# saiprasadbarke/robustmvd

Hardware: AMD Instinct MI355X
Metric: depth-maps/sec at 768x1152x4srcx256planes; warp+aggregate HBM GB/s vs roofline (higher is better)
Workload: dtype f32; 1 GPU; mvsnet (Path B) forward 768x1152, 4 source views, 256 planes, batch 1 per step (BASELINE.json configs[2]); the regulariser's two layers with 32 input channels (conv0, conv4): every fp32 operand as two range-scaled fp16 terms on fp16 MFMA, fp32 accumulation (at least as close to a float64 convolution as the fp32 matrix instruction over 1e-42..1e30: tests/test_hip_f16.py), the other nine layers and ; parallelism=1 independent replica(s), frames round-robin, no collectives

## Files before the change

### robustmvd_amd/csrc/conv2d_split.hip

```cpp
#include "mvd_common.h"
#include <algorithm>
#include <stdlib.h>

#ifndef C2_KO
#define C2_KO 0
#endif

namespace mvd {

typedef _Float16 c2h8 __attribute__((ext_vector_type(8)));
typedef float c2f4 __attribute__((ext_vector_type(4)));
typedef unsigned int c2u4 __attribute__((ext_vector_type(4)));
constexpr int C2_TH = 16, C2_TW = 16;

template <int KH, int KW, int S, int U8, bool IMG = false>
struct C2Geom {
    static constexpr int CC = 8 * U8;
    static constexpr int PB = 16;
    static constexpr int PH = (C2_TH - 1) * S + KH, PW = (C2_TW - 1) * S + KW;
    static constexpr int PWS = (PW + S - 1) / S;
    static constexpr int ROWB = S * S * PWS * PB;
    static constexpr int C8S = (PH * S * PWS * PB + 255) / 256 * 256;
    static constexpr int PLANE = U8 * C8S;
    static constexpr int UNITS = KH * KW * U8;
// ... 313 lines not shown
                xh = yh; xl = yl;
                if (m + 2 < MTW && !(C2_KO & 8)) {
                    yh = *reinterpret_cast<const c2h8*>(a + (m + 2) * G::ROWB);
                    yl = *reinterpret_cast<const c2h8*>(a + (m + 2) * G::ROWB + PLANE);
                }
#pragma unroll
                for (int t = 0; t < NTW; ++t) {
                    if (C2_KO & 2) {
                        acc[m][t][0] += (float)ch[0] * (float)wh[t][0] + (float)cl[1] * (float)wl[t][1];
                        continue;
                    }
                    acc[m][t] = __builtin_amdgcn_mfma_f32_16x16x32_f16(wh[t], ch, acc[m][t], 0, 0, 0);
                    acc[m][t] = __builtin_amdgcn_mfma_f32_16x16x32_f16(wl[t], ch, acc[m][t], 0, 0, 0);
                    acc[m][t] = __builtin_amdgcn_mfma_f32_16x16x32_f16(wh[t], cl, acc[m][t], 0, 0, 0);
                }
                __builtin_amdgcn_sched_barrier(0);
            }
#pragma unroll
            for (int t = 0; t < NTW; ++t) { wh[t] = nh[t]; wl[t] = nl[t]; }
        }
    }

    const int ox = ox0 + px16;
    float amax = 0.f;
#pragma unroll
    for (int t = 0; t < NTW; ++t) {
        const int cb = (nt0 + t) * 16 + 4 * g;
        if (p.part) {
            if (ox < p.Wo)
#pragma unroll
                for (int m = 0; m < MTW; ++m) {
                    const int oy = oy0 + wm * MTW + m;
                    if (oy >= p.Ho) continue;
                    const size_t pl = ((size_t)b * p.Ho + oy) * p.Wo + ox;
                    *reinterpret_cast<c2f4*>(p.part + (((size_t)cls * p.ksplit + ks) * p.B * p.Ho * p.Wo + pl) * p.ncp + cb) = acc[m][t];
                }
            continue;
        }
        if (cb >= p.Cout || ((C2_KO & 16) && p.B > 1000)) continue;
        const C2Chan kc = c2_chan(p, cb, xsc_inv);
        if (ox < p.Wo) {
            const size_t o0 = c2_out_offset(p, bb, od, oy0 + wm * MTW, ox, cls, cb), ostep = c2_row_step(p);
#pragma unroll
            for (int m = 0; m < MTW; ++m)
                if (oy0 + wm * MTW + m < p.Ho) c2_finish(p, o0 + m * ostep, cb, acc[m][t], kc, amax);
        }
    }
    if (p.yamax && !p.part) {
        for (int o = 32; o > 0; o >>= 1) amax = fmaxf(amax, __shfl_xor(amax, o));
        if (lane == 0) wmax[wv] = amax;
        __syncthreads();
        if (tid == 0) {
            amax = fmaxf(fmaxf(wmax[0], wmax[1]), fmaxf(wmax[2], wmax[3]));
            raise_absmax_seen(p.yamax, amax, amax_seen);
        }
    }
}

__global__ void __launch_bounds__(256) c2_reduce_kernel(C2Params p) {
    __shared__ float wmax[4];
    const int npix = p.B * p.Ho * p.Wo;
    const int c4n = (p.Cout + 3) / 4;
    const int cls = blockIdx.y;
    float xsc_inv;
    {
        const unsigned mb = __float_as_uint(*p.xamax);
        const int ex = (int)((mb >> 23) & 0xffu) - 127;
        const int e = max(-125, min(125, ex - 14));
        xsc_inv = __uint_as_float((unsigned)(127 + e) << 23);
    }
    float amax = 0.f;
    for (int i = blockIdx.x * 256 + threadIdx.x; i < npix * c4n; i += gridDim.x * 256) {
        const int pl = i / c4n;
        const int cb = (i - pl * c4n) * 4;
        const float* pp = p.part + ((size_t)cls * p.ksplit * npix + pl) * p.ncp + cb;
        const size_t kstr = (size_t)npix * p.ncp;
        c2f4 s = c2f4{0, 0, 0, 0};
        int ks = 0;
        for (; ks + 8 <= p.ksplit; ks += 8) {
            c2f4 v[8];
#pragma unroll
            for (int q = 0; q < 8; ++q) v[q] = *reinterpret_cast<const c2f4*>(pp + (size_t)(ks + q) * kstr);
#pragma unroll
            for (int q = 0; q < 8; ++q) s += v[q];
        }
        for (; ks + 2 <= p.ksplit; ks += 2) {
            const c2f4 v0 = *reinterpret_cast<const c2f4*>(pp + (size_t)ks * kstr), v1 = *reinterpret_cast<const c2f4*>(pp + (size_t)(ks + 1) * kstr);
            s += v0;
            s += v1;
        }
        const int row = pl / p.Wo, ox = pl - row * p.Wo, b = row / p.Ho, oy = row - b * p.Ho;
        const int bb = p.Do == 1 ? b : b / p.Do, od = b - bb * p.Do;
        c2_finish(p, c2_out_offset(p, bb, od, oy, ox, cls, cb), cb, s, c2_chan(p, cb, xsc_inv), amax);
    }
    if (p.yamax) {
        for (int o = 32; o > 0; o >>= 1) amax = fmaxf(amax, __shfl_xor(amax, o));
        if ((threadIdx.x & 63) == 0) wmax[threadIdx.x >> 6] = amax;
        __syncthreads();
        if (threadIdx.x == 0) {
            amax = fmaxf(fmaxf(wmax[0], wmax[1]), fmaxf(wmax[2], wmax[3]));
            raise_absmax(p.yamax, amax);
        }
    }
}

__global__ void __launch_bounds__(256) upsample2x_nhwc_kernel(const float* __restrict__ x, float* __restrict__ y, float* yamax, int B, int C, int h,
                                                              int w, int ys) {
    __shared__ float wmax[4];
    const long long n = (long long)B * 4 * h * w;
    float amax = 0.f;
    for (long long i = (long long)blockIdx.x * 256 + threadIdx.x; i < n; i += (long long)gridDim.x * 256) {
        const int ox = (int)(i % (2 * w)), oy = (int)((i / (2 * w)) % (2 * h)), b = (int)(i / (4LL * h * w));
        const float sy = fmaxf(0.5f * ((float)oy + 0.5f) - 0.5f, 0.f), sx = fmaxf(0.5f * ((float)ox + 0.5f) - 0.5f, 0.f);
        const int y0 = (int)sy, x0 = (int)sx;
        const int y1 = y0 + (y0 < h - 1 ? 1 : 0), x1 = x0 + (x0 < w - 1 ? 1 : 0);
        const float ly1 = sy - (float)y0, ly0 = 1.f - ly1, lx1 = sx - (float)x0, lx0 = 1.f - lx1;
        for (int c = 0; c < C; ++c) {
            const float* pl = x + ((size_t)b * C + c) * h * w;
            const float v = ly0 * (lx0 * pl[(size_t)y0 * w + x0] + lx1 * pl[(size_t)y0 * w + x1]) +
                            ly1 * (lx0 * pl[(size_t)y1 * w + x0] + lx1 * pl[(size_t)y1 * w + x1]);
            y[(size_t)i * ys + c] = v;
            amax = fmaxf(amax, finite_abs_or_zero(v));
        }
    }
    if (yamax) {
        for (int o = 32; o > 0; o >>= 1) amax = fmaxf(amax, __shfl_xor(amax, o));
        if ((threadIdx.x & 63) == 0) wmax[threadIdx.x >> 6] = amax;
        __syncthreads();
        if (threadIdx.x == 0) {
            amax = fmaxf(fmaxf(wmax[0], wmax[1]), fmaxf(wmax[2], wmax[3]));
            raise_absmax(yamax, amax);
        }
    }
}

__device__ __forceinline__ int c3_deconv_kidx(int a, int t) { return a == 0 ? (t == 0 ? 1 : -1) : (t == 0 ? 2 : 0); }

__global__ void c3_pack_kernel(const float* __restrict__ w, const float* __restrict__ eun, _Float16* __restrict__ packed, int Cin, int Cout,
                               int U8, int nchunks_c, int ntiles, int steps, int transposed, long long total) {
    const long long e = (long long)blockIdx.x * 256 + threadIdx.x;
    if (e >= total) return;
    const int KD = transposed ? 2 : 3, KP = transposed ? 2 : 3;
    const int j = (int)(e & 7), lane = (int)((e >> 3) & 63), term = (int)((e >> 9) & 1);
    long long r = e >> 10;
    const int step = (int)(r % steps); r /= steps;
    const int chunk = (int)(r % (KD * nchunks_c)); r /= KD * nchunks_c;
    const int nt = (int)r;
    const int kd = chunk / nchunks_c, cc = chunk % nchunks_c;
    const int ce = nt * 16 + (lane & 15), unit = 4 * step + (lane >> 4);
    const int tap = unit / U8, cin = cc * 8 * U8 + 8 * (unit % U8) + j;
    const int ncout = transposed ? 8 * Cout : Cout;
    float v = 0.f;
    if (tap < KP * KP && cin < Cin && ce < ncout) {
        const int ty = tap / KP, tx = tap % KP;
        if (transposed) {
            const int k3 = ce / Cout, c = ce % Cout;
            const int kz = c3_deconv_kidx(k3 >> 2, kd), ky = c3_deconv_kidx((k3 >> 1) & 1, ty), kx = c3_deconv_kidx(k3 & 1, tx);
            if (kz >= 0 && ky >= 0 && kx >= 0) v = w[((((size_t)cin * Cout + c) * 3 + kz) * 3 + ky) * 3 + kx];
        } else {
            v = w[((((size_t)ce * Cin + cin) * 3 + kd) * 3 + ty) * 3 + tx];
        }
        v = v / eun[ce];
    }
    const _Float16 hi = (_Float16)v;
    packed[e] = term == 0 ? hi : (_Float16)(v - (float)hi);
}

__global__ void c3_wscale_kernel(const float* __restrict__ w, float* __restrict__ eun, int Cin, int Cout, int transposed, int ncout, int cpad) {
    __shared__ float red[256];
    const int ce = blockIdx.x, c = ce % Cout;
    float m = 0.f;
    if (ce < ncout)
        for (int e = threadIdx.x; e < Cin * 27; e += 256) {
            const int ci = e / 27, t = e % 27;
            const float v = fabsf(transposed ? w[((size_t)ci * Cout + c) * 27 + t] : w[((size_t)c * Cin + ci) * 27 + t]);
            m = (v <= 3.4e38f && v > m) ? v : m;
        }
    red[threadIdx.x] = m;
    __syncthreads();
    for (int o = 128; o > 0; o >>= 1) {
        if (threadIdx.x < o) red[threadIdx.x] = fmaxf(red[threadIdx.x], red[threadIdx.x + o]);
        __syncthreads();
    }
    if (threadIdx.x == 0 && ce < cpad) {
        const int ex = (int)((__float_as_uint(red[0]) >> 23) & 0xffu) - 127;
        const int k = red[0] > 0.f ? max(-100, min(100, ex - 10)) : 0;
        eun[ce] = ldexpf(1.0f, k);
    }
}

struct C2Shape {
    int KH, KW, S, U8, steps;
    bool transposed, nchw3;
};

static bool c2_shape(int KH, int KW, int stride, int mode, int cin_pad, C2Shape* s) {
    s->transposed = mode == 1;
    s->nchw3 = mode == 2;
    s->KH = KH; s->KW = KW; s->S = stride;
    if (mode == 1) {
        if (KH != 4 || KW != 4 || stride != 2 || cin_pad % 32) return false;
        s->KH = s->KW = 2; s->S = 1; s->U8 = 4;
    } else if (mode == 2) {
        if (KH != 7 || KW != 7 || stride != 2 || cin_pad != 8) return false;
        s->U8 = 1;
        s->steps = 7;
        return true;
    } else if (KH == 1 && KW == 1 && stride == 1) {
        if (cin_pad % 32) return false;
        s->U8 = 4;
    } else if (KH == 3 && KW == 3 && stride == 1) {
        s->U8 = cin_pad % 32 == 0 ? 4 : 1;
    } else if ((KH == 3 && KW == 3 && stride == 2) || (KH == 5 && KW == 5 && stride == 2)) {
        s->U8 = 1;
    } else {
        return false;
    }
    if (cin_pad % (8 * s->U8)) return false;
    s->steps = (s->KH * s->KW * s->U8 + 3) / 4;
    return true;
}

static int c2_bn(int cout) {
    if (const char* e = exp_env("MVD_C2_BN")) {
        const int v = atoi(e);
        if (v == 16 || v == 32 || v == 64 || v == 128) return v;
    }
    return cout > 64 ? 128 : cout > 32 ? 64 : cout > 16 ? 32 : 16;
}
static int c2_ntiles(int cout) { return (cout + c2_bn(cout) - 1) / c2_bn(cout) * (c2_bn(cout) / 16); }
static size_t c2_frag_bytes(const C2Shape& s, int cin_pad, int cout) {
    const size_t nchunks = (size_t)cin_pad / (8 * s.U8);
    return (s.transposed ? 4 : 1) * (size_t)c2_ntiles(cout) * nchunks * s.steps * 2048;
}
static int c2_cpad(int cout) { return (cout + 127) / 128 * 128; }

struct C2Plan {
    int Ho, Wo, tiles_x, tiles_y, bn, nblocks, ncp, ncls, nchunks, ksplit;
    long long tiles;
    size_t part_bytes;
};
static C2Plan c2_plan(const C2Shape& s, int B, int Hi, int Wi, int cin_pad, int cout, int KH, int KW, int stride) {
    C2Plan q{};
    if (s.transposed) { q.Ho = Hi; q.Wo = Wi; q.ncls = 4; }
    else { q.Ho = (Hi + 2 * (KH / 2) - KH) / stride + 1; q.Wo = (Wi + 2 * (KW / 2) - KW) / stride + 1; q.ncls = 1; }
    q.tiles_y = (q.Ho + C2_TH - 1) / C2_TH;
    q.tiles_x = (q.Wo + C2_TW - 1) / C2_TW;
    q.bn = c2_bn(cout);
    q.nblocks = (cout + q.bn - 1) / q.bn;
    q.ncp = q.nblocks * q.bn;
    q.nchunks = cin_pad / (8 * s.U8);
    q.tiles = (long long)q.tiles_x * q.tiles_y * B * q.nblocks * q.ncls;
    q.ksplit = 1;
    if (q.tiles < 128)
        while (q.tiles * q.ksplit < 320 && q.ksplit < 32 && q.nchunks / (q.ksplit * 2) >= 2) q.ksplit *= 2;
    if (const char* e = exp_env("MVD_C2_KSPLIT")) {
        const int v = atoi(e);
        if (v >= 1 && v <= 32 && (v & (v - 1)) == 0 && v <= q.nchunks) q.ksplit = v;
    }
    q.part_bytes = q.ksplit > 1 ? (size_t)q.ksplit * q.ncls * B * q.Ho * q.Wo * q.ncp * sizeof(float) : 0;
    return q;
}

template <int KH, int KW, int S, int U8, int WM, int NTW, bool NCHW3>
static int c2_launch(const C2Params& p, long long nblk, hipStream_t st) {
    using G = C2Geom<KH, KW, S, U8, NCHW3>;
    auto kern = conv2d_split_kernel<KH, KW, S, U8, WM, NTW, NCHW3>;
    constexpr int lds = 2 * G::PLANE + 16;
    static_assert(lds <= 80 * 1024, "two workgroups per CU");
    if (lds > 48 * 1024 && hipFuncSetAttribute((const void*)kern, hipFuncAttributeMaxDynamicSharedMemorySize, lds) != hipSuccess)
        return launch_status("conv2d_split: LDS attribute");
    hipLaunchKernelGGL(kern, dim3((unsigned)nblk), dim3(256), lds, st, p);
    return launch_status("conv2d_split");
}

template <int KH, int KW, int S, int U8, bool NCHW3>
static int c2_launch_bn(const C2Params& p, int bn, long long nblk, hipStream_t st) {
    switch (bn) {
        case 128: return c2_launch<KH, KW, S, U8, 1, 2, NCHW3>(p, nblk, st);
        case 64: return c2_launch<KH, KW, S, U8, 1, 1, NCHW3>(p, nblk, st);
        case 32: return c2_launch<KH, KW, S, U8, 2, 1, NCHW3>(p, nblk, st);
        case 16: return c2_launch<KH, KW, S, U8, 4, 1, NCHW3>(p, nblk, st);
    }
    return MVD_ERR_INVALID_ARG;
}

static int c2_dispatch(const C2Shape& s, const C2Params& p, int bn, long long nblk, hipStream_t st) {
    if (s.nchw3) return c2_launch_bn<7, 7, 2, 1, true>(p, bn, nblk, st);
    if (s.KH == 1) return c2_launch_bn<1, 1, 1, 4, false>(p, bn, nblk, st);
    if (s.KH == 2) return s.U8 == 4 ? c2_launch_bn<2, 2, 1, 4, false>(p, bn, nblk, st) : c2_launch_bn<2, 2, 1, 2, false>(p, bn, nblk, st);
    if (s.KH == 5) return c2_launch_bn<5, 5, 2, 1, false>(p, bn, nblk, st);
    if (s.S == 2) return c2_launch_bn<3, 3, 2, 1, false>(p, bn, nblk, st);
    if (s.U8 == 4) return c2_launch_bn<3, 3, 1, 4, false>(p, bn, nblk, st);
    return c2_launch_bn<3, 3, 1, 1, false>(p, bn, nblk, st);
}

}

extern "C" {

size_t mvd_conv2d_split_packed_weight_bytes(int Cin_pad, int Cout, int KH, int KW, int stride, int mode) {
    mvd::C2Shape s;
    if (Cin_pad <= 0 || Cout <= 0 || !mvd::c2_shape(KH, KW, stride, mode, Cin_pad, &s)) return 0;
    return mvd::c2_frag_bytes(s, Cin_pad, Cout) + (size_t)mvd::c2_cpad(Cout) * sizeof(float);
}

int mvd_pack_conv2d_weights_split(const float* w, int Cin, int Cin_pad, int Cout, int KH, int KW, int stride, int mode, void* packed,
                                  mvd_stream_t stream) {
    MVD_REQUIRE(w && packed, "pack_conv2d_weights_split: NULL argument");
    mvd::C2Shape s;
    MVD_REQUIRE(Cin > 0 && Cin <= Cin_pad && Cout > 0 && mvd::c2_shape(KH, KW, stride, mode, Cin_pad, &s),
                "pack_conv2d_weights_split: layer %dx%d stride %d mode %d with %d (padded %d) -> %d channels is not built", KH, KW, stride, mode,
                Cin, Cin_pad, Cout);
    hipStream_t st = (hipStream_t)stream;
    const size_t fb = mvd::c2_frag_bytes(s, Cin_pad, Cout);
    float* eun = reinterpret_cast<float*>(static_cast<char*>(packed) + fb);
    const int cpad = mvd::c2_cpad(Cout);
    hipLaunchKernelGGL(mvd::c2_wscale_kernel, dim3(cpad), dim3(256), 0, st, w, eun, Cin, Cout, KH * KW, s.transposed ? 1 : 0, cpad);
    const long long total = (long long)(fb / 2);
    hipLaunchKernelGGL(mvd::c2_pack_kernel, dim3((unsigned)((total + 255) / 256)), dim3(256), 0, st, w, eun, (_Float16*)packed, Cin, Cout, s.KH,
                       s.KW, s.U8, Cin_pad / (8 * s.U8), mvd::c2_ntiles(Cout), s.steps, s.transposed ? 1 : s.nchw3 ? 2 : 0, total);
    return mvd::launch_status("pack_conv2d_weights_split");
}

size_t mvd_conv2d_split_workspace_bytes(int B, int Hi, int Wi, int Cin_pad, int Cout, int KH, int KW, int stride, int mode) {
    mvd::C2Shape s;
    if (B <= 0 || Hi <= 0 || Wi <= 0 || Cin_pad <= 0 || Cout <= 0 || !mvd::c2_shape(KH, KW, stride, mode, Cin_pad, &s)) return 0;
    return mvd::c2_plan(s, B, Hi, Wi, Cin_pad, Cout, KH, KW, stride).part_bytes;
}

int mvd_conv2d_split_f32(const float* x, const float* x_absmax, const void* packed_w, const float* bias, float* y, float* y_absmax, int B,
                         int Hi, int Wi, int Cin_pad, int x_pixel_stride, int Cout, int y_pixel_stride, long long y_row_stride,
                         long long y_image_stride, long long y_channel_stride, int KH, int KW, int stride, int mode, int act, float slope,
                         void* workspace, size_t workspace_bytes, mvd_stream_t stream) {
    MVD_REQUIRE(x && x_absmax && packed_w && y, "conv2d_split: NULL argument");
    MVD_REQUIRE(B > 0 && Hi > 0 && Wi > 0, "conv2d_split: non-positive dimension");
    mvd::C2Shape s;
    MVD_REQUIRE(Cin_pad > 0 && Cout > 0 && mvd::c2_shape(KH, KW, stride, mode, Cin_pad, &s),
                "conv2d_split: layer %dx%d stride %d mode %d with %d -> %d channels is not built", KH, KW, stride, mode, Cin_pad, Cout);
    MVD_REQUIRE(mode == 2 || (x_pixel_stride >= Cin_pad && x_pixel_stride % 4 == 0), "conv2d_split: input pixel stride %d (channels %d)",
                x_pixel_stride, Cin_pad);
    if (y_channel_stride <= 0) y_channel_stride = 1;
    MVD_REQUIRE(y_channel_stride != 1 || y_pixel_stride >= Cout, "conv2d_split: output pixel stride %d below %d channels", y_pixel_stride, Cout);
    MVD_REQUIRE(y_pixel_stride >= 1 && y_row_stride >= 0 && y_image_stride >= 0, "conv2d_split: negative output stride");
    MVD_REQUIRE(act >= 0 && act <= 2, "conv2d_split: act=%d unknown", act);
    MVD_REQUIRE(mode == 2 || (((uintptr_t)x & 15) == 0 && ((uintptr_t)y & 15) == 0), "conv2d_split: x and y must be 16-byte aligned");
    hipStream_t st = (hipStream_t)stream;
    mvd::C2Params p{};
    p.x = x; p.xamax = x_absmax; p.bias = bias; p.y = y; p.yamax = y_absmax;
    p.B = B; p.Hi = Hi; p.Wi = Wi; p.xs = x_pixel_stride; p.nchunks = Cin_pad / (8 * s.U8);
    p.Di = p.Do = p.Dy = p.KD = p.SD = 1; p.pad_d = 0; p.nchunks_c = p.nchunks; p.sub3d = 0; p.Cr = Cout;
    p.Cout = Cout; p.ys = y_pixel_stride; p.act = act; p.slope = slope;
    const size_t fb = mvd::c2_frag_bytes(s, Cin_pad, Cout);
    p.eun = reinterpret_cast<const float*>(static_cast<const char*>(packed_w) + fb);
    const mvd::C2Plan q = mvd::c2_plan(s, B, Hi, Wi, Cin_pad, Cout, KH, KW, stride);
    p.Ho = q.Ho; p.Wo = q.Wo; p.ncls = q.ncls;
    if (s.transposed) {
        p.Hy = 2 * Hi; p.Wy = 2 * Wi; p.oy_mul = p.ox_mul = 2; p.pad_y = p.pad_x = 1;
    } else {
        p.Hy = p.Ho; p.Wy = p.Wo; p.oy_mul = p.ox_mul = 1; p.pad_y = KH / 2; p.pad_x = KW / 2;
    }
    MVD_REQUIRE(y_channel_stride != 1 || Cout < 4 || (y_pixel_stride % 4 == 0 && y_row_stride % 4 == 0 && y_image_stride % 4 == 0),
                "conv2d_split: channel-last output strides must be multiples of 4 floats");
    p.ycs = y_channel_stride;
    p.ys_row = y_row_stride > 0 ? y_row_stride : (long long)p.Wy * y_pixel_stride;
    p.ys_img = y_image_stride > 0 ? y_image_stride : (long long)p.Hy * p.ys_row;
    p.wpk = static_cast<const char*>(packed_w);
    p.cls_bytes = (long long)(fb / p.ncls);
    p.tiles_y = q.tiles_y; p.tiles_x = q.tiles_x;
    const int bn = q.bn;
    p.nblocks = q.nblocks;
    p.ncp = q.ncp;
    const long long tiles = q.tiles;
    int ksplit = q.ksplit;
    if (ksplit > 1 && (!workspace || workspace_bytes < q.part_bytes)) ksplit = 1;
    p.ksplit = ksplit;
    p.chunks_per_split = (p.nchunks + ksplit - 1) / ksplit;
    p.part = ksplit > 1 ? static_cast<float*>(workspace) : nullptr;
    const long long nblk = tiles * ksplit;
    MVD_REQUIRE(nblk <= 0x7fffffffLL, "conv2d_split: %lld workgroups exceed the grid limit", nblk);
    int rc = mvd::c2_dispatch(s, p, bn, nblk, st);
    if (rc != MVD_OK || ksplit == 1) return rc;
    const long long n = (long long)B * p.Ho * p.Wo * ((Cout + 3) / 4);
    MVD_REQUIRE(n < 0x7fffffffLL, "conv2d_split: split reduction over %lld outputs", n);
    hipLaunchKernelGGL(mvd::c2_reduce_kernel, dim3((unsigned)std::min<long long>((n + 255) / 256, 1024), (unsigned)p.ncls), dim3(256), 0, st, p);
    return mvd::launch_status("conv2d_split: reduce");
}

int mvd_upsample2x_nhwc_f32(const float* x, float* y, float* y_absmax, int B, int C, int h, int w, int y_pixel_stride, mvd_stream_t stream) {
    MVD_REQUIRE(x && y, "upsample2x_nhwc: NULL argument");
    MVD_REQUIRE(B > 0 && C > 0 && h > 0 && w > 0 && y_pixel_stride >= C, "upsample2x_nhwc: bad dimension");
    const long long n = (long long)B * 4 * h * w;
    hipLaunchKernelGGL(mvd::upsample2x_nhwc_kernel, dim3((unsigned)std::min<long long>((n + 255) / 256, 1024)), dim3(256), 0, (hipStream_t)stream, x, y,
                       y_absmax, B, C, h, w, y_pixel_stride);
    return mvd::launch_status("upsample2x_nhwc");
}

}

namespace mvd {
static bool c3_shape(int Cin, int Cout, int mode, C2Shape* s, int* ncout) {
    if (Cin <= 0 || Cin % 8 || Cout <= 0 || Cout % 4 || mode < 0 || mode > 2) return false;
    s->transposed = false; s->nchw3 = false;
    if (mode == MVD_DECONV3D_STRIDE2) {
        if (Cin % 16) return false;
        s->KH = s->KW = 2; s->S = 1; s->U8 = Cin % 32 == 0 ? 4 : 2;
        *ncout = 8 * Cout;
    } else {
        s->KH = s->KW = 3; s->S = mode == MVD_CONV3D_STRIDE2 ? 2 : 1;
        s->U8 = (s->S == 1 && Cin % 32 == 0) ? 4 : 1;
        *ncout = Cout;
    }
    s->steps = (s->KH * s->KW * s->U8 + 3) / 4;
    return true;
}
static size_t c3_frag_bytes(const C2Shape& s, int Cin, int ncout, int mode) {
    const size_t KD = mode == MVD_DECONV3D_STRIDE2 ? 2 : 3;
    return (size_t)c2_ntiles(ncout) * KD * (Cin / (8 * s.U8)) * s.steps * 2048;
}
}

extern "C" {

size_t mvd_conv3d_igemm_packed_weight_bytes(int Cin, int Cout, int mode) {
    mvd::C2Shape s;
    int ncout;
    if (!mvd::c3_shape(Cin, Cout, mode, &s, &ncout)) return 0;
    return mvd::c3_frag_bytes(s, Cin, ncout, mode) + (size_t)mvd::c2_cpad(ncout) * sizeof(float);
}

int mvd_pack_conv3d_weights_igemm(const float* w, int Cin, int Cout, int mode, void* packed, mvd_stream_t stream) {
    MVD_REQUIRE(w && packed, "pack_conv3d_weights_igemm: NULL argument");
    mvd::C2Shape s;
    int ncout;
    MVD_REQUIRE(mvd::c3_shape(Cin, Cout, mode, &s, &ncout), "pack_conv3d_weights_igemm: %d -> %d channels, mode %d is not built", Cin, Cout, mode);
    hipStream_t st = (hipStream_t)stream;
    const size_t fb = mvd::c3_frag_bytes(s, Cin, ncout, mode);
    float* eun = reinterpret_cast<float*>(static_cast<char*>(packed) + fb);
    const int cpad = mvd::c2_cpad(ncout), tr = mode == MVD_DECONV3D_STRIDE2 ? 1 : 0;
    hipLaunchKernelGGL(mvd::c3_wscale_kernel, dim3(cpad), dim3(256), 0, st, w, eun, Cin, Cout, tr, ncout, cpad);
    const long long total = (long long)(fb / 2);
    hipLaunchKernelGGL(mvd::c3_pack_kernel, dim3((unsigned)((total + 255) / 256)), dim3(256), 0, st, w, eun, (_Float16*)packed, Cin, Cout, s.U8,
                       Cin / (8 * s.U8), mvd::c2_ntiles(ncout), s.steps, tr, total);
    return mvd::launch_status("pack_conv3d_weights_igemm");
}

static mvd::C2Plan c3_plan(const mvd::C2Shape& s, int B, int Di, int Hi, int Wi, int Cin, int ncout, int mode, int* Do) {
    mvd::C2Plan q{};
    const int sd = mode == MVD_CONV3D_STRIDE2 ? 2 : 1;
    *Do = Di / sd; q.Ho = Hi / sd; q.Wo = Wi / sd; q.ncls = 1;
    q.tiles_y = (q.Ho + mvd::C2_TH - 1) / mvd::C2_TH;
    q.tiles_x = (q.Wo + mvd::C2_TW - 1) / mvd::C2_TW;
    q.bn = mvd::c2_bn(ncout);
    q.nblocks = (ncout + q.bn - 1) / q.bn;
    q.ncp = q.nblocks * q.bn;
    q.nchunks = (mode == MVD_DECONV3D_STRIDE2 ? 2 : 3) * (Cin / (8 * s.U8));
    q.tiles = (long long)q.tiles_x * q.tiles_y * B * *Do * q.nblocks;
    q.ksplit = 1;
    if (q.tiles < 128)
        while (q.tiles * q.ksplit < 320 && q.ksplit < 32 && q.nchunks / (q.ksplit * 2) >= 2) q.ksplit *= 2;
    q.part_bytes = q.ksplit > 1 ? (size_t)q.ksplit * B * *Do * q.Ho * q.Wo * q.ncp * sizeof(float) : 0;
    return q;
}

size_t mvd_conv3d_igemm_workspace_bytes(int B, int Di, int Hi, int Wi, int Cin, int Cout, int mode) {
    mvd::C2Shape s;
    int ncout, Do;
    if (B <= 0 || Di <= 0 || Hi <= 0 || Wi <= 0 || !mvd::c3_shape(Cin, Cout, mode, &s, &ncout)) return 0;
    return c3_plan(s, B, Di, Hi, Wi, Cin, ncout, mode, &Do).part_bytes;
}

int mvd_conv3d_bn_relu_igemm_f32(const float* x, const float* x_absmax, const void* packed_w, const float* scale, const float* shift,
                                 const float* skip, float* y, float* y_absmax, int B, int Di, int Hi, int Wi, int Cin, int Cout, int mode,
                                 int relu, void* workspace, size_t workspace_bytes, mvd_stream_t stream) {
    MVD_REQUIRE(x && x_absmax && packed_w && scale && shift && y, "conv3d_igemm: NULL argument");
    MVD_REQUIRE(B > 0 && Di > 0 && Hi > 0 && Wi > 0, "conv3d_igemm: non-positive dimension");
    mvd::C2Shape s;
    int ncout;
    MVD_REQUIRE(mvd::c3_shape(Cin, Cout, mode, &s, &ncout), "conv3d_igemm: %d -> %d channels, mode %d is not built", Cin, Cout, mode);
    MVD_REQUIRE(mode != MVD_CONV3D_STRIDE2 || (Di % 2 == 0 && Hi % 2 == 0 && Wi % 2 == 0), "conv3d_igemm stride 2: odd input dims %dx%dx%d", Di, Hi, Wi);
    MVD_REQUIRE((((uintptr_t)x | (uintptr_t)y | (uintptr_t)skip) & 15) == 0, "conv3d_igemm: x, y and skip must be 16-byte aligned");
    hipStream_t st = (hipStream_t)stream;
    int Do;
    const mvd::C2Plan q = c3_plan(s, B, Di, Hi, Wi, Cin, ncout, mode, &Do);
    const bool tr = mode == MVD_DECONV3D_STRIDE2;
    mvd::C2Params p{};
    p.x = x; p.xamax = x_absmax; p.bias = shift; p.scale = scale; p.skip = skip; p.y = y; p.yamax = y_absmax;
    p.wpk = static_cast<const char*>(packed_w);
    p.eun = reinterpret_cast<const float*>(p.wpk + mvd::c3_frag_bytes(s, Cin, ncout, mode));
    p.B = B * Do; p.Hi = Hi; p.Wi = Wi; p.xs = Cin; p.nchunks = q.nchunks;
    p.Di = Di; p.Do = Do; p.KD = tr ? 2 : 3; p.SD = mode == MVD_CONV3D_STRIDE2 ? 2 : 1; p.pad_d = tr ? 0 : 1; p.nchunks_c = Cin / (8 * s.U8);
    p.sub3d = tr ? 1 : 0; p.Cr = Cout; p.Dy = tr ? 2 * Di : Do;
    p.Ho = q.Ho; p.Wo = q.Wo; p.Hy = tr ? 2 * Hi : q.Ho; p.Wy = tr ? 2 * Wi : q.Wo;
    p.oy_mul = p.ox_mul = 1; p.pad_y = p.pad_x = tr ? 0 : 1;
    p.Cout = ncout; p.ncp = q.ncp; p.ys = Cout; p.ycs = 1;
    p.ys_row = (long long)p.Wy * Cout; p.ys_img = (long long)p.Hy * p.ys_row;
    p.tiles_x = q.tiles_x; p.tiles_y = q.tiles_y; p.nblocks = q.nblocks; p.ncls = 1; p.cls_bytes = 0;
    p.act = relu ? 2 : 0; p.slope = 0.f;
    int ksplit = q.ksplit;
    if (ksplit > 1 && (!workspace || workspace_bytes < q.part_bytes)) ksplit = 1;
    p.ksplit = ksplit;
    p.chunks_per_split = (p.nchunks + ksplit - 1) / ksplit;
    p.part = ksplit > 1 ? static_cast<float*>(workspace) : nullptr;
    const long long nblk = q.tiles * ksplit;
    MVD_REQUIRE(nblk <= 0x7fffffffLL, "conv3d_igemm: %lld workgroups exceed the grid limit", nblk);
    int rc = mvd::c2_dispatch(s, p, q.bn, nblk, st);
    if (rc != MVD_OK || ksplit == 1) return rc;
    const long long n = (long long)p.B * p.Ho * p.Wo * ((p.Cout + 3) / 4);
    MVD_REQUIRE(n < 0x7fffffffLL, "conv3d_igemm: split reduction over %lld outputs", n);
    hipLaunchKernelGGL(mvd::c2_reduce_kernel, dim3((unsigned)std::min<long long>((n + 255) / 256, 1024)), dim3(256), 0, st, p);
    return mvd::launch_status("conv3d_igemm: reduce");
}
}
```

### robustmvd_amd/csrc/mvd_common.h

```cpp
#pragma once
#include <hip/hip_runtime.h>
#include <stdarg.h>
#include <stdio.h>

#include "mvd.h"

namespace mvd {

void set_error(const char* fmt, ...);
void timing_begin(hipStream_t st);
void timing_end(hipStream_t st);
int absmax_launch(const float* x, long long n, float* absmax, hipStream_t st);
__device__ __forceinline__ void raise_absmax(float* slot, float m) {
    if (m > 0.f && m > __builtin_nontemporal_load(slot)) atomicMax(reinterpret_cast<unsigned*>(slot), __float_as_uint(m));
}
__device__ __forceinline__ float absmax_seen(const float* slot) { return slot ? __builtin_nontemporal_load(slot) : 0.f; }
__device__ __forceinline__ void raise_absmax_seen(float* slot, float m, float seen) {
    if (m > seen) raise_absmax(slot, m);
}
__device__ __forceinline__ float finite_abs_or_zero(float v) {
    const float a = fabsf(v);
    return a <= 3.402823466e38f ? a : 0.f;
}

bool conv3d_c1_ok(int Cout);
int conv3d_c1_pack(const float* w, int Cout, float* packed, hipStream_t st);
int conv3d_c1_launch(const float* x, const float* packed_w, const float* scale, const float* shift, const float* skip, float* y, int B,
                     int D, int h, int w, int Cout, int relu, hipStream_t st);

inline int launch_status(const char* what) {
    hipError_t e = hipGetLastError();
    if (e != hipSuccess) {
        set_error("%s: %s", what, hipGetErrorString(e));
        return MVD_ERR_LAUNCH;
    }
    return MVD_OK;
}

#define MVD_REQUIRE(cond, ...)          \
    do {                                \
        if (!(cond)) {                  \
            mvd::set_error(__VA_ARGS__); \
            return MVD_ERR_INVALID_ARG; \
        }                               \
    } while (0)

struct ViewPtrs {
    const float* p[MVD_MAX_VIEWS];
};
struct ViewOutPtrs {
    float* p[MVD_MAX_VIEWS];
};

inline size_t align_up(size_t x, size_t a) { return (x + a - 1) / a * a; }

#ifdef MVD_EXPERIMENTS
const char* exp_env(const char* name);
#else
constexpr const char* exp_env(const char*) { return nullptr; }
#endif

__device__ __forceinline__ float unnormalize_coord(float g, float size) {
    return ((g + 1.0f) * size - 1.0f) / 2.0f;
}

struct Taps {
    int off[4];
    float w[4];
    float inb;
};

__device__ __forceinline__ Taps bilinear_taps(float ix, float iy, int hs, int ws) {
    Taps t;
    const float x0 = floorf(ix), y0 = floorf(iy);
    const float x1 = x0 + 1.0f, y1 = y0 + 1.0f;
    const float wx1 = ix - x0, wx0 = x1 - ix, wy1 = iy - y0, wy0 = y1 - iy;
    const float xs[4] = {x0, x1, x0, x1};
    const float ys[4] = {y0, y0, y1, y1};
    const float wt[4] = {wx0 * wy0, wx1 * wy0, wx0 * wy1, wx1 * wy1};
    const float xmax = (float)(ws - 1), ymax = (float)(hs - 1);
    t.inb = 0.0f;
#pragma unroll
    for (int k = 0; k < 4; ++k) {
        const bool in = (xs[k] >= 0.0f) && (xs[k] <= xmax) && (ys[k] >= 0.0f) && (ys[k] <= ymax);
        t.off[k] = in ? ((int)ys[k] * ws + (int)xs[k]) : 0;
        t.w[k] = in ? wt[k] : 0.0f;
        t.inb += t.w[k];
    }
    return t;
}

}
```

Measured before the change: 318.0 depth-maps/sec.

## Add row-streaming split-fp16 MFMA kernel for 3x3 stride-1 16/32-channel convs

Adds a dedicated conv2d kernel for 3x3 stride-1 layers with 16 or 32 equal in/out channels. Each wave owns a 16-pixel column strip and streams down a band of rows. It keeps the split-fp16 weights in registers and rotates three accumulators, so each input row is loaded and split once and feeds all three kernel rows. The next row is prefetched while the current one runs. This replaces the generic tiled split kernel's shared-memory patch staging for these layers, at the cost of extra packed-weight storage, a second pack launch and high register pressure.

```diff
diff --git a/robustmvd_amd/csrc/conv2d_rows.hip b/robustmvd_amd/csrc/conv2d_rows.hip
--- /dev/null
+++ b/robustmvd_amd/csrc/conv2d_rows.hip
@@ -0,0 +1,232 @@
+#include "mvd_common.h"
+#include <algorithm>
+#include <stdlib.h>
+
+namespace mvd {
+
+typedef _Float16 crh8 __attribute__((ext_vector_type(8)));
+typedef float crf4 __attribute__((ext_vector_type(4)));
+typedef unsigned int cru4 __attribute__((ext_vector_type(4)));
+
+struct C2RowsParams {
+    const float* x;
+    const float* xamax;
+    const char* wpk;
+    const float* eun;
+    const float* bias;
+    float* y;
+    float* yamax;
+    int B, H, W, xs, ys;
+    long long ys_row, ys_img;
+    int rpw, nseg;
+    int tiles_x, nblk, blk_per_xcd;
+    int relu;
+};
+
+template <int C>
+struct C2RowsGeom {
+    static constexpr int NS = C == 16 ? 2 : 3;
+    static constexpr int NT = C / 16;
+    static constexpr int SPB = 4 / NT;
+    static constexpr size_t FRAG_BYTES = (size_t)NT * 3 * NS * 2 * 1024;
+};
+
+__global__ void c2rows_pack_kernel(const float* __restrict__ w, const float* __restrict__ eun, _Float16* __restrict__ packed, int Cin, int C,
+                                   int total) {
+    const int e = blockIdx.x * 256 + threadIdx.x;
+    if (e >= total) return;
+    const int NS = C == 16 ? 2 : 3;
+    const int j = e & 7, lane = (e >> 3) & 63, term = (e >> 9) & 1;
+    int r = e >> 10;
+    const int s = r % NS; r /= NS;
+    const int kh = r % 3;
+    const int nt = r / 3;
+    const int cout = nt * 16 + (lane & 15), q = lane >> 4;
+    const int kw = C == 16 ? 2 * s + (q >> 1) : s, cin = C == 16 ? 8 * (q & 1) + j : 8 * q + j;
+    float v = 0.f;
+    if (kw < 3 && cin < Cin) v = w[(((size_t)cout * Cin + cin) * 3 + kh) * 3 + kw] / eun[cout];
+    const _Float16 hi = (_Float16)v;
+    packed[e] = term == 0 ? hi : (_Float16)(v - (float)hi);
+}
+
+template <int C>
+__global__ void __launch_bounds__(256, C == 16 ? 3 : 2) conv2d_rows_kernel(C2RowsParams p) {
+    using G = C2RowsGeom<C>;
+    constexpr int NS = G::NS, NT = G::NT, SPB = G::SPB;
+    constexpr unsigned OOB = 0x80000000u;
+    __shared__ float wmax[4];
+    const float amax_seen = absmax_seen(p.yamax);
+    const int lane = threadIdx.x & 63, wv = __builtin_amdgcn_readfirstlane(threadIdx.x >> 6);
+    const int q = lane >> 4, px = lane & 15;
+
+    const int blk = (blockIdx.x & 7) * p.blk_per_xcd + (blockIdx.x >> 3);
+    if (blk >= p.nblk) return;
+    const int tx = blk % p.tiles_x, seg = (blk / p.tiles_x) % p.nseg, b = blk / (p.tiles_x * p.nseg);
+    const int nt = wv % NT, x0 = (tx * SPB + wv / NT) * 16;
+    const int r0 = seg * p.rpw, r1 = min(r0 + p.rpw, p.H);
+
+    float amax = 0.f;
+    if (x0 < p.W) {
+        float xsc, xsc_inv;
+        {
+            const unsigned mb = __builtin_amdgcn_readfirstlane((int)__float_as_uint(*p.xamax));
+            const int ex = (int)((mb >> 23) & 0xffu) - 127;
+            const int e = max(-125, min(125, ex - 14));
+            xsc = __uint_as_float((unsigned)(127 - e) << 23);
+            xsc_inv = __uint_as_float((unsigned)(127 + e) << 23);
+        }
+        const float one = 1.0f;
+        auto split2 = [xsc, one](float a0, float a1, unsigned& hi, unsigned& lo) {
+            unsigned hp, lp;
+            float t0, t1;
+            asm("v_fma_mixlo_f16 %0, %1, %2, 0 op_sel:[0,0,0] op_sel_hi:[0,0,0]" : "=v"(hp) : "v"(a0), "s"(xsc));
+            asm("v_fma_mixhi_f16 %0, %1, %2, 0 op_sel:[0,0,0] op_sel_hi:[0,0,0]" : "+v"(hp) : "v"(a1), "s"(xsc));
+            asm("v_fma_mix_f32 %0, %1, %2, -%3 op_sel:[0,0,0] op_sel_hi:[0,0,1]" : "=v"(t0) : "v"(a0), "s"(xsc), "v"(hp));
+            asm("v_fma_mix_f32 %0, %1, %2, -%3 op_sel:[0,0,1] op_sel_hi:[0,0,1]" : "=v"(t1) : "v"(a1), "s"(xsc), "v"(hp));
+            asm("v_fma_mixlo_f16 %0, %1, %2, 0 op_sel:[0,0,0] op_sel_hi:[0,0,0]" : "=v"(lp) : "v"(t0), "s"(one));
+            asm("v_fma_mixhi_f16 %0, %1, %2, 0 op_sel:[0,0,0] op_sel_hi:[0,0,0]" : "+v"(lp) : "v"(t1), "s"(one));
+            hi = hp;
+            lo = lp;
+        };
+
+        crh8 wh[3][NS], wl[3][NS];
+        {
+            const char* wlane = p.wpk + (size_t)nt * 3 * NS * 2048 + lane * 16;
+#pragma unroll
+            for (int kh = 0; kh < 3; ++kh)
+#pragma unroll
+                for (int s = 0; s < NS; ++s) {
+                    wh[kh][s] = *reinterpret_cast<const crh8*>(wlane + (kh * NS + s) * 2048);
+                    wl[kh][s] = *reinterpret_cast<const crh8*>(wlane + (kh * NS + s) * 2048 + 1024);
+                }
+        }
+        unsigned xoff[NS];
+#pragma unroll
+        for (int s = 0; s < NS; ++s) {
+            const int kw = C == 16 ? 2 * s + (q >> 1) : s, c8 = C == 16 ? (q & 1) : q;
+            const int col = x0 + px - 1 + kw;
+            xoff[s] = (kw < 3 && col >= 0 && col < p.W) ? (unsigned)((col * p.xs + 8 * c8) * 4) : OOB;
+        }
+        const int cb = nt * 16 + 4 * q;
+        const unsigned yoff = x0 + px < p.W ? (unsigned)(((x0 + px) * p.ys + cb) * 4) : OOB;
+        float mul[4], bi[4];
+#pragma unroll
+        for (int r = 0; r < 4; ++r) {
+            mul[r] = p.eun[cb + r] * xsc_inv;
+            bi[r] = p.bias ? p.bias[cb + r] : 0.f;
+        }
+        const float* xim = p.x + (size_t)b * p.H * p.W * p.xs;
+        float* yim = p.y + (size_t)b * p.ys_img;
+        const size_t xrow = (size_t)p.W * p.xs;
+        const int xrow_bytes = ((p.W - 1) * p.xs + C) * 4, yrow_bytes = ((p.W - 1) * p.ys + C) * 4;
+
+        cru4 raw[NS][2];
+        auto fetch = [&](int r, bool ok) {
+            const __amdgpu_buffer_rsrc_t rs =
+                __builtin_amdgcn_make_buffer_rsrc(const_cast<float*>(xim + (ok ? (size_t)r * xrow : 0)), 0, ok ? xrow_bytes : 0, 0x00020000);
+#pragma unroll
+            for (int s = 0; s < NS; ++s) {
+                raw[s][0] = __builtin_amdgcn_raw_buffer_load_b128(rs, xoff[s], 0, 0);
+                raw[s][1] = __builtin_amdgcn_raw_buffer_load_b128(rs, xoff[s] + 16u, 0, 0);
+            }
+        };
+        auto finish = [&](const crf4& a, int orow, bool ok) {
+            const __amdgpu_buffer_rsrc_t rs = __builtin_amdgcn_make_buffer_rsrc(yim + (ok ? (size_t)orow * p.ys_row : 0), 0, ok ? yrow_bytes : 0, 0x00020000);
+            float v[4];
+#pragma unroll
+            for (int r = 0; r < 4; ++r) {
+                v[r] = a[r] * mul[r] + bi[r];
+                if (p.relu) v[r] = fmaxf(v[r], 0.f);
+                amax = fmaxf(amax, (ok && yoff != OOB) ? finite_abs_or_zero(v[r]) : 0.f);
+            }
+            __builtin_amdgcn_raw_buffer_store_b128(cru4{__float_as_uint(v[0]), __float_as_uint(v[1]), __float_as_uint(v[2]), __float_as_uint(v[3])},
+                                                   rs, yoff, 0, 0);
+        };
+
+        const int rlo = max(r0 - 1, 0), rhi = min(r1, p.H - 1);
+        crf4 acc[3] = {crf4{0, 0, 0, 0}, crf4{0, 0, 0, 0}, crf4{0, 0, 0, 0}};
+        fetch(rlo, true);
+        for (int r = rlo; r <= rhi; ++r) {
+            crh8 fh[NS], fl[NS];
+#pragma unroll
+            for (int s = 0; s < NS; ++s) {
+                cru4 hv, lv;
+#pragma unroll
+                for (int k = 0; k < 4; ++k) {
+                    const crf4 v = __builtin_bit_cast(crf4, raw[s][k >> 1]);
+                    unsigned hi, lo;
+                    split2(v[(k & 1) * 2], v[(k & 1) * 2 + 1], hi, lo);
+                    hv[k] = hi; lv[k] = lo;
+                }
+                fh[s] = __builtin_bit_cast(crh8, hv);
+                fl[s] = __builtin_bit_cast(crh8, lv);
+            }
+            fetch(r + 1, r + 1 <= rhi);
+            __builtin_amdgcn_sched_barrier(0);
+#pragma unroll
+            for (int s = 0; s < NS; ++s) {
+#pragma unroll
+                for (int i = 0; i < 3; ++i) acc[i] = __builtin_amdgcn_mfma_f32_16x16x32_f16(wh[2 - i][s], fh[s], acc[i], 0, 0, 0);
+#pragma unroll
+                for (int i = 0; i < 3; ++i) acc[i] = __builtin_amdgcn_mfma_f32_16x16x32_f16(wl[2 - i][s], fh[s], acc[i], 0, 0, 0);
+#pragma unroll
+                for (int i = 0; i < 3; ++i) acc[i] = __builtin_amdgcn_mfma_f32_16x16x32_f16(wh[2 - i][s], fl[s], acc[i], 0, 0, 0);
+            }
+            finish(acc[0], r - 1, r - 1 >= r0);
+            acc[0] = acc[1];
+            acc[1] = acc[2];
+            acc[2] = crf4{0, 0, 0, 0};
+        }
+        finish(acc[0], rhi, rhi < r1);
+    }
+    if (p.yamax) {
+        for (int o = 32; o > 0; o >>= 1) amax = fmaxf(amax, __shfl_xor(amax, o));
+        if (lane == 0) wmax[wv] = amax;
+        __syncthreads();
+        if (threadIdx.x == 0) {
+            amax = fmaxf(fmaxf(wmax[0], wmax[1]), fmaxf(wmax[2], wmax[3]));
+            raise_absmax_seen(p.yamax, amax, amax_seen);
+        }
+    }
+}
+
+bool conv2d_rows_ok(int Cin_pad, int Cout, int KH, int KW, int stride, int mode) {
+    return mode == 0 && KH == 3 && KW == 3 && stride == 1 && Cin_pad == Cout && (Cout == 16 || Cout == 32);
+}
+
+size_t conv2d_rows_frag_bytes(int C) { return C == 16 ? C2RowsGeom<16>::FRAG_BYTES : C2RowsGeom<32>::FRAG_BYTES; }
+
+int conv2d_rows_pack(const float* w, const float* eun, int Cin, int C, void* frag, hipStream_t st) {
+    const int total = (int)(conv2d_rows_frag_bytes(C) / 2);
+    hipLaunchKernelGGL(c2rows_pack_kernel, dim3((unsigned)((total + 255) / 256)), dim3(256), 0, st, w, eun, (_Float16*)frag, Cin, C, total);
+    return launch_status("pack_conv2d_weights_split: rows");
+}
+
+bool conv2d_rows_fits(int B, int H, int W, int xs, int ys) {
+    return (long long)W * xs * 4 < 0x7fffffffLL && (long long)W * ys * 4 < 0x7fffffffLL && (long long)B * H * ((W + 15) / 16) < 0x3fffffffLL;
+}
+
+int conv2d_rows_launch(const float* x, const float* xamax, const void* frag, const float* eun, const float* bias, float* y, float* yamax, int B,
+                       int H, int W, int C, int xs, int ys, long long ys_row, long long ys_img, int relu, hipStream_t st) {
+    C2RowsParams p{};
+    p.x = x; p.xamax = xamax; p.wpk = static_cast<const char*>(frag); p.eun = eun; p.bias = bias; p.y = y; p.yamax = yamax;
+    p.B = B; p.H = H; p.W = W; p.xs = xs; p.ys = ys; p.ys_row = ys_row; p.ys_img = ys_img; p.relu = relu;
+    const int spb = C == 16 ? C2RowsGeom<16>::SPB : C2RowsGeom<32>::SPB;
+    p.tiles_x = (W + 16 * spb - 1) / (16 * spb);
+    int rpw = 32;
+    while (rpw > 4 && (long long)B * p.tiles_x * ((H + rpw - 1) / rpw) < 4096) rpw /= 2;
+    if (const char* e = exp_env("MVD_C2_ROWS_RPW")) {
+        const int v = atoi(e);
+        if (v >= 1 && v <= 4096) rpw = v;
+    }
+    p.rpw = rpw;
+    p.nseg = (H + rpw - 1) / rpw;
+    p.nblk = B * p.nseg * p.tiles_x;
+    p.blk_per_xcd = (p.nblk + 7) / 8;
+    const dim3 grid((unsigned)(8 * p.blk_per_xcd));
+    if (C == 16) hipLaunchKernelGGL(conv2d_rows_kernel<16>, grid, dim3(256), 0, st, p);
+    else hipLaunchKernelGGL(conv2d_rows_kernel<32>, grid, dim3(256), 0, st, p);
+    return launch_status("conv2d_split: rows");
+}
+
+}
diff --git a/robustmvd_amd/csrc/conv2d_split.hip b/robustmvd_amd/csrc/conv2d_split.hip
--- a/robustmvd_amd/csrc/conv2d_split.hip
+++ b/robustmvd_amd/csrc/conv2d_split.hip
@@ -639,7 +639,8 @@
 size_t mvd_conv2d_split_packed_weight_bytes(int Cin_pad, int Cout, int KH, int KW, int stride, int mode) {
     mvd::C2Shape s;
     if (Cin_pad <= 0 || Cout <= 0 || !mvd::c2_shape(KH, KW, stride, mode, Cin_pad, &s)) return 0;
-    return mvd::c2_frag_bytes(s, Cin_pad, Cout) + (size_t)mvd::c2_cpad(Cout) * sizeof(float);
+    return mvd::c2_frag_bytes(s, Cin_pad, Cout) + (size_t)mvd::c2_cpad(Cout) * sizeof(float) +
+           (mvd::conv2d_rows_ok(Cin_pad, Cout, KH, KW, stride, mode) ? mvd::conv2d_rows_frag_bytes(Cout) : 0);
 }
 
 int mvd_pack_conv2d_weights_split(const float* w, int Cin, int Cin_pad, int Cout, int KH, int KW, int stride, int mode, void* packed,
@@ -657,6 +658,8 @@
     const long long total = (long long)(fb / 2);
     hipLaunchKernelGGL(mvd::c2_pack_kernel, dim3((unsigned)((total + 255) / 256)), dim3(256), 0, st, w, eun, (_Float16*)packed, Cin, Cout, s.KH,
                        s.KW, s.U8, Cin_pad / (8 * s.U8), mvd::c2_ntiles(Cout), s.steps, s.transposed ? 1 : s.nchw3 ? 2 : 0, total);
+    if (mvd::conv2d_rows_ok(Cin_pad, Cout, KH, KW, stride, mode))
+        return mvd::conv2d_rows_pack(w, eun, Cin, Cout, eun + cpad, st);
     return mvd::launch_status("pack_conv2d_weights_split");
 }
 
@@ -690,6 +693,18 @@
     p.Cout = Cout; p.ys = y_pixel_stride; p.act = act; p.slope = slope;
     const size_t fb = mvd::c2_frag_bytes(s, Cin_pad, Cout);
     p.eun = reinterpret_cast<const float*>(static_cast<const char*>(packed_w) + fb);
+    if (mvd::conv2d_rows_ok(Cin_pad, Cout, KH, KW, stride, mode) && y_channel_stride == 1 && act != 1 &&
+        mvd::conv2d_rows_fits(B, Hi, Wi, x_pixel_stride, y_pixel_stride)) {
+        const char* e = mvd::exp_env("MVD_C2_ROWS");
+        if (!e || atoi(e) != 0) {
+            MVD_REQUIRE(y_pixel_stride % 4 == 0 && y_row_stride % 4 == 0 && y_image_stride % 4 == 0,
+                        "conv2d_split: channel-last output strides must be multiples of 4 floats");
+            const long long ys_row = y_row_stride > 0 ? y_row_stride : (long long)Wi * y_pixel_stride;
+            const long long ys_img = y_image_stride > 0 ? y_image_stride : (long long)Hi * ys_row;
+            return mvd::conv2d_rows_launch(x, x_absmax, p.eun + mvd::c2_cpad(Cout), p.eun, bias, y, y_absmax, B, Hi, Wi, Cout, x_pixel_stride,
+                                           y_pixel_stride, ys_row, ys_img, act == 2, st);
+        }
+    }
     const mvd::C2Plan q = mvd::c2_plan(s, B, Hi, Wi, Cin_pad, Cout, KH, KW, stride);
     p.Ho = q.Ho; p.Wo = q.Wo; p.ncls = q.ncls;
     if (s.transposed) {
diff --git a/robustmvd_amd/csrc/mvd_common.h b/robustmvd_amd/csrc/mvd_common.h
--- a/robustmvd_amd/csrc/mvd_common.h
+++ b/robustmvd_amd/csrc/mvd_common.h
@@ -27,6 +27,13 @@
 int conv3d_c1_pack(const float* w, int Cout, float* packed, hipStream_t st);
 int conv3d_c1_launch(const float* x, const float* packed_w, const float* scale, const float* shift, const float* skip, float* y, int B,
                      int D, int h, int w, int Cout, int relu, hipStream_t st);
+
+bool conv2d_rows_ok(int Cin_pad, int Cout, int KH, int KW, int stride, int mode);
+bool conv2d_rows_fits(int B, int H, int W, int xs, int ys);
+size_t conv2d_rows_frag_bytes(int C);
+int conv2d_rows_pack(const float* w, const float* eun, int Cin, int C, void* frag, hipStream_t st);
+int conv2d_rows_launch(const float* x, const float* xamax, const void* frag, const float* eun, const float* bias, float* y, float* yamax, int B,
+                       int H, int W, int C, int xs, int ys, long long ys_row, long long ys_img, int relu, hipStream_t st);
 
 inline int launch_status(const char* what) {
     hipError_t e = hipGetLastError();
```

Result: no change. 315.1 depth-maps/sec (-0.9%).
